# brentp/goleft

Measured on AMD Instinct MI355X. Metric: ref bases/sec per-base depth, 30x WGS synthetic, higher is better.
Workload: dtype int32; 1 GPU; synthetic 30x WGS, hg19 contig lengths (3.1 Gb), 150 bp reads; window=1000, min_mapq=1, min_cov=4, total_ref_bases=3095677412, reads_rank0=619135482, cigar_ops_rank0=687232250, canonical_cigar_ops_rank0=0, tiles_on_the_generic_kernel=24, step=gd_compute on the records as they arrived (nothing derived exists), outputs=int32 per-base depth + int64/int32 window sum/min + class runs, tile_positions=4096, lookback=192

## Files before the change

### goleft_amd/csrc/gd_kernels.hpp

```cpp
#pragma once

#include <hip/hip_runtime.h>
#include <stdint.h>

namespace gd {

constexpr int WAVE = 64;
constexpr int SUPER = 1024;

struct ContigDev {
    const int32_t*  pos;
    const uint16_t* flag;
    const uint8_t*  mapq;
    const uint32_t* off;
    const uint32_t* cigar;
    uint32_t n_reads;
    uint32_t n_ops;
    int32_t  length;
    int32_t  tile_beg;
    int32_t  n_tiles;
    int64_t  base_off;
    int64_t  win_off;
    int32_t  tid;
    uint32_t unit_beg;
    uint32_t grp_beg;
    const uint4*    lrec;
    const uint32_t* lfq;
    const uint2*    dl;
    const uint32_t* pck;
    const uint32_t* ndel;
    const uint32_t* rec;
    const uint32_t* pidx;
    uint32_t pidx_last;
    uint32_t pad_;
};

struct __attribute__((aligned(16))) TileInfo {
    const int32_t*  pos;
    const uint16_t* flag;
    const uint8_t*  mapq;
    const uint32_t* off;
    const uint32_t* cigar;
    int64_t  base_off;
    int64_t  win_off;
    int32_t  length;
    int32_t  ctg;
    int32_t  t0;
    uint32_t lo, hi;
    uint32_t n_reads;
    uint32_t n_ops;
    uint32_t clo, chi;
    int32_t  tile;
    int32_t  pad_;
    const uint32_t* ndel;
    const uint4*    lrec;
    const uint32_t* lfq;
    const uint2*    dl;
    const uint32_t* pck;
};

struct __attribute__((aligned(16))) TileFast {
    const int32_t*  pos;
    const uint32_t* rec;
    const uint32_t* cig;
    const uint16_t* flag;
    const uint8_t*  mapq;
    int32_t*  out;
    int64_t*  wsum;
    int32_t*  wmin;
    int32_t   t0;
    uint32_t  nrd;
    uint32_t  nst;
    uint32_t  clo;
    int32_t   ctg;
    int32_t   pad_[3];
    uint32_t  win0[4];
    int32_t   wleft[4];
    int32_t   sleft[4];
};
constexpr int FAST_BIG = 0x3fffffff;
constexpr int FAST_FAR = FAST_BIG - 65536;

struct Counters {
    int32_t  max_span;
    uint32_t run_cursor;
    uint32_t pad0;
    uint32_t pad1;
    uint32_t n_slow[2];
    uint32_t pad2[2];
};

struct Job {
    const ContigDev* ctgs;
    int32_t   n_ctgs;
    int32_t   n_tiles;
    TileInfo* tiles;
    int32_t*  perbase;
    int64_t*  win_sum;
    int32_t*  win_min;
    int64_t   n_win_total;
    int2*     run_chunks;
    uint32_t  run_cap;
    uint32_t* tile_cnt;
    uint32_t* tile_off;
    uint32_t* super_cnt;
    Counters* counters;
    int32_t   W;
    int32_t   Q;
    int32_t   mincov;
    int32_t   maxmean;
    uint32_t  flag_mask;
    int32_t   lookback;
    int32_t   reserved0;
    int64_t   step;
    uint32_t  n_units;
    uint32_t  n_groups;
    unsigned long long* tile_status;
    uint32_t  w_magic, w_shift;
    uint32_t  s_magic, s_shift;
    uint32_t  fast;
    uint32_t  parity;
    TileFast* ftiles;
};

__device__ __forceinline__ int cov_class(int d, int mincov, int maxmean)
{
    int c = 2;
    if (maxmean > 0 && d >= maxmean) c = 3;
    if (d < mincov) c = 1;
    if (d == 0) c = 0;
    return c;
}

__device__ __forceinline__ uint32_t lower_bound_i32(const int32_t* a, uint32_t n, int32_t key)
{
    uint32_t lo = 0, hi = n;
    while (lo < hi) {
        uint32_t mid = lo + ((hi - lo) >> 1);
        if (a[mid] < key) lo = mid + 1; else hi = mid;
    }
    return lo;
}

__device__ __forceinline__ void lower_bound_pair(const int32_t* a, uint32_t n, int32_t keyA,
                                                 int32_t keyB, uint32_t& outA, uint32_t& outB)
{
    uint32_t la = 0, ha = n, lb = 0, hb = n;
    if (n == 0) { outA = 0; outB = 0; return; }
    const uint32_t last = n - 1;
    while (ha > la || hb > lb) {
        const uint32_t wa = ha - la, wb = hb - lb;
        uint32_t a1 = la + (wa >> 2), a2 = la + (wa >> 1), a3 = la + wa - (wa >> 2) - (wa != 0);
        uint32_t b1 = lb + (wb >> 2), b2 = lb + (wb >> 1), b3 = lb + wb - (wb >> 2) - (wb != 0);
        a1 = a1 < last ? a1 : last; a2 = a2 < last ? a2 : last; a3 = a3 < last ? a3 : last;
        b1 = b1 < last ? b1 : last; b2 = b2 < last ? b2 : last; b3 = b3 < last ? b3 : last;
        const int32_t va1 = a[a1], va2 = a[a2], va3 = a[a3];
        const int32_t vb1 = a[b1], vb2 = a[b2], vb3 = a[b3];
        if (wa != 0) {
            if (va3 < keyA) la = a3 + 1;
            else if (va2 < keyA) { la = a2 + 1; ha = a3; }
            else if (va1 < keyA) { la = a1 + 1; ha = a2; }
            else ha = a1;
        }
        if (wb != 0) {
            if (vb3 < keyB) lb = b3 + 1;
            else if (vb2 < keyB) { lb = b2 + 1; hb = b3; }
            else if (vb1 < keyB) { lb = b1 + 1; hb = b2; }
            else hb = b1;
        }
    }
    outA = la;
    outB = lb;
}

__device__ __forceinline__ uint32_t lower_bound_hint(const int32_t* a, uint32_t n, int32_t key, uint32_t guess)
{
    if (n == 0u) return 0u;
    constexpr uint32_t R = 8192u;
    const uint32_t g = guess < n ? guess : n - 1u;
    const uint32_t pl = g > R ? g - R : 0u;
    const uint32_t ph = n - 1u - g > R ? g + R : n - 1u;
    const int32_t vl = a[pl], vh = a[ph];
    uint32_t lo = 0, hi = n;
    if (vl < key) {
        lo = pl + 1u;
        if (vh >= key) hi = ph; else lo = ph + 1u;
    } else {
        hi = pl;
    }
    while (lo < hi) {
        const uint32_t mid = lo + ((hi - lo) >> 1);
        if (a[mid] < key) lo = mid + 1u; else hi = mid;
    }
    return lo;
}

template <int T>
__global__ void gd_prep_kernel(Job job)
{
    const int64_t gid = (int64_t)blockIdx.x * blockDim.x + threadIdx.x;
    const int64_t gsz = (int64_t)gridDim.x * blockDim.x;
    for (int64_t w = gid; w < job.n_win_total; w += gsz) {
        job.win_sum[w] = 0;
        job.win_min[w] = 0x7fffffff;
    }
    for (int64_t g = gid; g < (job.n_tiles + SUPER - 1) / SUPER; g += gsz) job.super_cnt[g] = 0;
    const int32_t lookback = job.lookback;
    if (gid == 0) {
        job.counters->max_span = 0;
        job.counters->run_cursor = 0;
        job.counters->n_slow[job.parity ^ 1u] = 0;
    }
    if (gid >= job.n_tiles) return;
    const int t = (int)gid;
    int lo = 0, hi = job.n_ctgs;
    while (hi - lo > 1) {
        int mid = (lo + hi) >> 1;
        if (job.ctgs[mid].tile_beg <= t) lo = mid; else hi = mid;
    }
    const ContigDev c = job.ctgs[lo];
    TileInfo ti;
    ti.pos = c.pos; ti.flag = c.flag; ti.mapq = c.mapq; ti.off = c.off; ti.cigar = c.cigar;
    ti.base_off = c.base_off; ti.win_off = c.win_off; ti.length = c.length;
    ti.n_reads = c.n_reads; ti.n_ops = c.n_ops;
    ti.ctg = lo;
    ti.tile = t;
    ti.pad_ = 0;
    ti.ndel = c.ndel;
    ti.lrec = c.lrec; ti.lfq = c.lfq; ti.dl = c.dl; ti.pck = c.pck;
    ti.t0 = (t - c.tile_beg) * T;
    int32_t tend = ti.t0 + T < c.length ? ti.t0 + T : c.length;
    int32_t from = ti.t0 > lookback ? ti.t0 - lookback : 0;
    if (c.pidx) {
        const uint32_t kl = (uint32_t)from >> 6, k = (uint32_t)tend >> 6;
        ti.lo = kl > c.pidx_last ? c.n_reads : c.pidx[kl];
        const uint32_t a = k > c.pidx_last ? c.n_reads : c.pidx[k];
        ti.hi = (tend & 63) == 0 ? a : a + lower_bound_i32(c.pos + a, (k + 1u > c.pidx_last ? c.n_reads : c.pidx[k + 1]) - a, tend);
    } else {
        const uint32_t n = c.n_reads;
        const uint32_t g0 = (uint32_t)(((uint64_t)(uint32_t)ti.t0 * n) / (uint32_t)c.length);
        const uint32_t s0 = ti.t0 == 0 ? 0u : lower_bound_hint(c.pos, n, ti.t0, g0);
        const uint32_t nxt = (uint32_t)__shfl_down((int)s0, 1, WAVE);
        const int tnx = __shfl_down(t, 1, WAVE);
        const bool have = (threadIdx.x & 63u) != 63u && t + 1 < job.n_tiles && tnx == t + 1 &&
                          t + 1 - c.tile_beg < c.n_tiles && ti.t0 + T == tend;
        if (have) ti.hi = nxt;
        else {
            const uint32_t g1 = (uint32_t)(((uint64_t)(uint32_t)tend * n) / (uint32_t)c.length);
            ti.hi = lower_bound_hint(c.pos + s0, n - s0, tend, g1 > s0 ? g1 - s0 : 0u) + s0;
        }
        uint32_t lo = 0, hi2 = s0;
        if (from == 0) hi2 = 0u;
        for (uint32_t step = 64u; hi2 > 0u; step <<= 2) {
            const uint32_t p = hi2 > step ? hi2 - step : 0u;
            if (c.pos[p] >= from) hi2 = p; else { lo = p + 1u; break; }
        }
        while (lo < hi2) {
            const uint32_t mid = lo + ((hi2 - lo) >> 1);
            if (c.pos[mid] < from) lo = mid + 1u; else hi2 = mid;
        }
        ti.lo = lo;
    }
    if (job.fast == 2u) ti.lo &= ~3u;
    ti.clo = c.n_reads ? c.off[ti.lo] : 0u;
    ti.chi = c.n_reads ? c.off[ti.hi] : 0u;
    if (!job.fast) { job.tiles[t] = ti; return; }
    TileFast tf;
    const uint32_t nrd = ti.hi - ti.lo, nst = ti.chi - ti.clo;
    const bool ordinary = tend - ti.t0 == T && nrd <= 1024u && nst <= (job.fast == 2u ? 1280u : 1024u);
    tf.nrd = 0xffffffffu;
    if (ordinary) {
        tf.pos = c.pos + ti.lo; tf.cig = c.cigar + ti.clo;
        if (job.fast == 2u) { tf.rec = c.off + ti.lo; tf.flag = c.flag + ti.lo; tf.mapq = c.mapq + ti.lo; }
        else { tf.rec = c.rec + ti.lo; tf.flag = nullptr; tf.mapq = nullptr; }
        tf.out = job.perbase ? job.perbase + c.base_off + ti.t0 : nullptr;
        tf.wsum = job.win_sum + c.win_off;
        tf.wmin = job.win_min + c.win_off;
        tf.t0 = ti.t0; tf.nrd = nrd; tf.nst = nst; tf.clo = ti.clo; tf.ctg = lo;
        tf.pad_[0] = tf.pad_[1] = tf.pad_[2] = 0;
        const uint32_t W = (uint32_t)job.W;
        const uint32_t stepc = job.step > 0x7fffffffLL ? 0x7fffffffu : (uint32_t)job.step;
#pragma unroll
        for (int w = 0; w < 4; ++w) {
            const uint32_t cpos0 = (uint32_t)ti.t0 + (uint32_t)(w * (T / 4));
            const uint32_t cw = cpos0 / W, wleft = W - (cpos0 - cw * W);
            const uint32_t srem = cpos0 % stepc, sleft = srem == 0u ? 0u : stepc - srem;
            tf.win0[w] = cw;
            tf.wleft[w] = wleft > (uint32_t)FAST_FAR ? FAST_BIG : (int32_t)wleft;
            tf.sleft[w] = sleft > (uint32_t)FAST_FAR ? FAST_BIG : (int32_t)sleft;
        }
    } else {
        const uint32_t slot = atomicAdd(&job.counters->n_slow[job.parity], 1u);
        job.tiles[slot] = ti;
    }
    job.ftiles[t] = tf;
}

__global__ __launch_bounds__(64) void gd_copy_words_kernel(const uint32_t* __restrict__ src, uint32_t* __restrict__ dst, uint32_t n)
{
    for (uint32_t i = threadIdx.x; i < n; i += 64u) dst[i] = src[i];
}

__global__ __launch_bounds__(256) void gd_readback_kernel(const Counters* __restrict__ k, const int2* __restrict__ ordered, uint32_t spec,
                                                          Counters* __restrict__ h_counters, int2* __restrict__ h_bounds)
{
    const uint32_t n = k->run_cursor < spec ? k->run_cursor : spec;
    for (uint32_t i = threadIdx.x; i < n; i += 256u) h_bounds[i] = ordered[i];
    if (threadIdx.x < sizeof(Counters) / 4u)
        reinterpret_cast<uint32_t*>(h_counters)[threadIdx.x] = reinterpret_cast<const uint32_t*>(k)[threadIdx.x];
}

__device__ __forceinline__ int wave_inclusive_scan(int v)
{
    v += __builtin_amdgcn_update_dpp(0, v, 0x111, 0xf, 0xf, false);
    v += __builtin_amdgcn_update_dpp(0, v, 0x112, 0xf, 0xf, false);
    v += __builtin_amdgcn_update_dpp(0, v, 0x114, 0xf, 0xf, false);
    v += __builtin_amdgcn_update_dpp(0, v, 0x118, 0xf, 0xf, false);
    v += __builtin_amdgcn_update_dpp(0, v, 0x142, 0xa, 0xf, false);
    v += __builtin_amdgcn_update_dpp(0, v, 0x143, 0xc, 0xf, false);
    return v;
}

__device__ __forceinline__ void scan4(int& a, int& b, int& c, int& d)
{
#define GD_DPP4(ctl)                                  \
    "v_add_u32_dpp %0, %0, %0 " ctl "\n\t"            \
    "v_add_u32_dpp %1, %1, %1 " ctl "\n\t"            \
    "v_add_u32_dpp %2, %2, %2 " ctl "\n\t"            \
    "v_add_u32_dpp %3, %3, %3 " ctl "\n\t"
    asm volatile(
        "s_nop 1\n\t"
        GD_DPP4("row_shr:1 row_mask:0xf bank_mask:0xf bound_ctrl:1")
        GD_DPP4("row_shr:2 row_mask:0xf bank_mask:0xf bound_ctrl:1")
        GD_DPP4("row_shr:4 row_mask:0xf bank_mask:0xf bound_ctrl:1")
        GD_DPP4("row_shr:8 row_mask:0xf bank_mask:0xf bound_ctrl:1")
        GD_DPP4("row_bcast:15 row_mask:0xa bank_mask:0xf")
        GD_DPP4("row_bcast:31 row_mask:0xc bank_mask:0xf")
        : "+v"(a), "+v"(b), "+v"(c), "+v"(d));
#undef GD_DPP4
}

__device__ __forceinline__ int wave_sum(int v)
{
#pragma unroll
    for (int m = 32; m >= 1; m >>= 1) v += __shfl_xor(v, m, WAVE);
    return v;
}

__device__ __forceinline__ long long wave_sum64(long long v)
{
#pragma unroll
    for (int m = 32; m >= 1; m >>= 1) v += __shfl_xor(v, m, WAVE);
    return v;
}

__device__ __forceinline__ int wave_min(int v)
{
#pragma unroll
    for (int m = 32; m >= 1; m >>= 1) {
        int o = __shfl_xor(v, m, WAVE);
        v = o < v ? o : v;
    }
    return v;
}

struct RegionTab {
    const int32_t* depth;
    int64_t  clen, start, end;
    int64_t  first_win;
    uint32_t win_off;
    uint32_t chunk_off;
};
constexpr int REGION_CHUNK = 4096;

__global__ __launch_bounds__(256) void gd_regions_windows_kernel(const RegionTab* __restrict__ tab,
                                                                 const uint32_t* __restrict__ win_region, int32_t W,
                                                                 int64_t* __restrict__ sums, int32_t* __restrict__ mins)
{
    __shared__ long long s_sum[4];
    __shared__ int s_min[4];
    const uint32_t w = blockIdx.x;
    const RegionTab t = tab[win_region[w]];
    const int64_t k = t.first_win + (int64_t)(w - t.win_off);
    int64_t ws = k * W, we = ws + W;
    if (ws < t.start) ws = t.start;
    if (we > t.end) we = t.end;
    long long acc = 0;
    int mn = 0x7fffffff;
    for (int64_t p = ws + threadIdx.x; p < we; p += 256) {
        const int d = p < t.clen ? t.depth[p] : 0;
        acc += d;
        mn = d < mn ? d : mn;
    }
    acc = wave_sum64(acc);
    mn = wave_min(mn);
    const int lane = threadIdx.x & 63, wv = threadIdx.x >> 6;
    if (lane == 0) { s_sum[wv] = acc; s_min[wv] = mn; }
    __syncthreads();
    if (threadIdx.x == 0) {
        int m = s_min[0];
        for (int i = 1; i < 4; ++i) m = s_min[i] < m ? s_min[i] : m;
        sums[w] = s_sum[0] + s_sum[1] + s_sum[2] + s_sum[3];
        mins[w] = m;
    }
}

__global__ __launch_bounds__(256) void gd_regions_bounds_kernel(const RegionTab* __restrict__ tab,
                                                                const uint32_t* __restrict__ chunk_region, int mincov,
                                                                int maxmean, int4* __restrict__ out, uint32_t cap,
                                                                uint32_t* __restrict__ cursor)
{
    const uint32_t ch = blockIdx.x;
    const uint32_t r = chunk_region[ch];
    const RegionTab t = tab[r];
    const int64_t p0 = t.start + (int64_t)(ch - t.chunk_off) * REGION_CHUNK;
    const int64_t p1 = p0 + REGION_CHUNK < t.end ? p0 + REGION_CHUNK : t.end;
    for (int64_t p = p0 + threadIdx.x; p < p1; p += 256) {
        const int d = p < t.clen ? t.depth[p] : 0;
        const int cl = cov_class(d, mincov, maxmean);
        bool b = (p == t.start);
        if (!b) {
            const int dp = (p - 1) < t.clen ? t.depth[p - 1] : 0;
// ... 144 lines not shown
```

### goleft_amd/csrc/gd_tile_common.hpp

```cpp
#pragma once

#include <type_traits>

namespace gd {

typedef __amdgpu_buffer_rsrc_t rsrc_t;

__device__ __forceinline__ rsrc_t make_rsrc(const void* p, uint32_t bytes)
{
    return __builtin_amdgcn_make_buffer_rsrc(const_cast<void*>(p), (short)0, (int)bytes, 0x00020000);
}

__device__ __forceinline__ int wave_total(int v)
{
    return __builtin_amdgcn_readlane(wave_inclusive_scan(v), 63);
}

__device__ __forceinline__ int wave_prev_lane(int v, int first)
{
    return __builtin_amdgcn_update_dpp(first, v, 0x138, 0xf, 0xf, false);
}

__device__ __forceinline__ int wave_min_dpp(int v)
{
    int o;
    o = __builtin_amdgcn_update_dpp(v, v, 0x111, 0xf, 0xf, false); v = o < v ? o : v;
    o = __builtin_amdgcn_update_dpp(v, v, 0x112, 0xf, 0xf, false); v = o < v ? o : v;
    o = __builtin_amdgcn_update_dpp(v, v, 0x114, 0xf, 0xf, false); v = o < v ? o : v;
    o = __builtin_amdgcn_update_dpp(v, v, 0x118, 0xf, 0xf, false); v = o < v ? o : v;
    o = __builtin_amdgcn_update_dpp(v, v, 0x142, 0xa, 0xf, false); v = o < v ? o : v;
    o = __builtin_amdgcn_update_dpp(v, v, 0x143, 0xc, 0xf, false); v = o < v ? o : v;
    return __builtin_amdgcn_readlane(v, 63);
}

__device__ __forceinline__ uint32_t wave_max_dpp(uint32_t v)
{
    uint32_t o;
    o = (uint32_t)__builtin_amdgcn_update_dpp((int)v, (int)v, 0x111, 0xf, 0xf, false); v = o > v ? o : v;
    o = (uint32_t)__builtin_amdgcn_update_dpp((int)v, (int)v, 0x112, 0xf, 0xf, false); v = o > v ? o : v;
    o = (uint32_t)__builtin_amdgcn_update_dpp((int)v, (int)v, 0x114, 0xf, 0xf, false); v = o > v ? o : v;
    o = (uint32_t)__builtin_amdgcn_update_dpp((int)v, (int)v, 0x118, 0xf, 0xf, false); v = o > v ? o : v;
    o = (uint32_t)__builtin_amdgcn_update_dpp((int)v, (int)v, 0x142, 0xa, 0xf, false); v = o > v ? o : v;
    o = (uint32_t)__builtin_amdgcn_update_dpp((int)v, (int)v, 0x143, 0xc, 0xf, false); v = o > v ? o : v;
    return (uint32_t)__builtin_amdgcn_readlane((int)v, 63);
}

__device__ __forceinline__ void publish_span(int32_t* max_span, uint32_t smax, int seen0, int lane)
{
    if (__builtin_amdgcn_ballot_w64(smax > (uint32_t)seen0) != 0ull) {
        const uint32_t m = wave_max_dpp(smax);
        if (lane == 0) atomicMax(max_span, (int32_t)m);
    }
}

__device__ __forceinline__ int32_t* lds_at(int32_t* base, int b4)
{
    return reinterpret_cast<int32_t*>(reinterpret_cast<char*>(base) + b4);
}

__device__ __forceinline__ void mark4(int32_t* s_diff, int s4, int e4, int T4)
{
    if (e4 >= 0) {
        const int cs4 = s4 > -4 ? s4 : -4;
        atomicAdd(lds_at(s_diff, cs4), 1);
        if (e4 < T4) atomicAdd(lds_at(s_diff, e4), -1);
    }
}

constexpr uint32_t SPAN_SAT = 1u << 28;

template <typename OpPtr>
__device__ __forceinline__ uint32_t walk_cigar4(OpPtr ops, uint32_t n, int ps4, int T4, int32_t* s_diff)
{
    uint32_t span = 0;
    for (uint32_t k = 0; k < n; ++k) {
        const uint32_t cg = ops[k];
        const uint32_t op = cg & 0xf, len = cg >> 4;
        const bool counted = (0x181u >> op) & 1u;
        const bool consumes = (0x18du >> op) & 1u;
        if (counted && len != 0 && span < SPAN_SAT) {
            const int s4 = ps4 + (int)(span << 2);
            if (s4 < T4) mark4(s_diff, s4, s4 + (int)(len << 2), T4);
        }
        if (consumes) { span += len; span = span < SPAN_SAT ? span : SPAN_SAT; }
    }
    return span;
}

struct PhaseA {
    const int32_t* pos; const uint16_t* flag; const uint8_t* mapq; const uint32_t* off;
    int32_t* s_diff;
    const uint32_t* s_cig;
    uint32_t* wq;
    const uint32_t* gcig;
    uint32_t clo, nrd;
    int neg4t0, T4;
    uint32_t flag_mask;
    int Q, tid, lane;
};

struct PhaseB {
    int32_t* s_diff;
    uint32_t* s_bmap; uint32_t* s_clo; uint32_t* s_chi; uint32_t* s_hasb;
    int32_t* out;
    int64_t* wsum; int32_t* wmin;
    int t0, tlen, chunk0, carry, lane;
    int W, mincov, maxmean;
    int64_t step;
};

template <int ROWS, bool FULL, bool WIDE, int ST>
__device__ __forceinline__ void phase_b_rows(const PhaseB& B)
{
    constexpr int BIG = 0x3fffffff;
    typedef typename std::conditional<WIDE, unsigned long long, uint32_t>::type acc_t;
    const int lane = B.lane, t0 = B.t0, tlen = B.tlen, chunk0 = B.chunk0;
    const int W = B.W;
    int carry = B.carry;

    const uint32_t cpos0 = (uint32_t)t0 + (uint32_t)chunk0;
    uint32_t cur_win = cpos0 / (uint32_t)W;
    const int64_t nb_abs = ((int64_t)cur_win + 1) * (int64_t)W;
    int nb = (nb_abs - t0) > BIG ? BIG : (int)(nb_abs - t0);
    const uint32_t stepc = B.step > 0x7fffffffLL ? 0x7fffffffu : (uint32_t)B.step;
    const int64_t nf_abs = (int64_t)((cpos0 + stepc - 1) / stepc) * (int64_t)stepc;
    int nf = (nf_abs - t0) > BIG ? BIG : (int)(nf_abs - t0);
    const int wstep = W > BIG ? BIG : W;
    const int fstep = stepc > (uint32_t)BIG ? BIG : (int)stepc;
    acc_t acc = 0;
    int mn = 0x7fffffff;
    const int lo_thr = B.mincov > 1 ? B.mincov : 1;
    const int hi_thr = B.maxmean > 0 ? B.maxmean : 0x7fffffff;
    const bool has_max = B.maxmean > 0;

#pragma unroll
    for (int r = 0; r < ROWS; ++r) {
        const int rb = chunk0 + r * 256;
        const int ib = rb + lane * 4;
        int4* dst = reinterpret_cast<int4*>(&B.out[ib]);
        if (!FULL && rb >= tlen) {
            if (ST != 2) *dst = make_int4(0, 0, 0, 0);
            continue;
        }
        const int4 v = *reinterpret_cast<const int4*>(&B.s_diff[ib]);
        const int x1 = v.x + v.y, x2 = x1 + v.z, x3 = x2 + v.w;
        const int incl = wave_inclusive_scan(x3);
        const int base = carry + (incl - x3);
        int d0 = base + v.x, d1 = base + x1, d2 = base + x2, d3 = base + x3;
        const int carry_before = carry;
        carry += __builtin_amdgcn_readlane(incl, 63);
        int nvalid = 4;
        if (!FULL) {
            nvalid = tlen - ib;
            nvalid = nvalid < 0 ? 0 : (nvalid > 4 ? 4 : nvalid);
            d0 = nvalid > 0 ? d0 : 0; d1 = nvalid > 1 ? d1 : 0;
            d2 = nvalid > 2 ? d2 : 0; d3 = nvalid > 3 ? d3 : 0;
        }
        if (ST == 2) {
        } else if (ST == 1) {
            typedef int v4i32 __attribute__((ext_vector_type(4)));
            v4i32 dv; dv.x = d0; dv.y = d1; dv.z = d2; dv.w = d3;
            __builtin_nontemporal_store(dv, reinterpret_cast<v4i32*>(dst));
        } else {
            *dst = make_int4(d0, d1, d2, d3);
        }

        const uint32_t s4 = (uint32_t)d0 + (uint32_t)d1 + (uint32_t)d2 + (uint32_t)d3;
        int t = d0 < d1 ? d0 : d1;
        t = d2 < t ? d2 : t;
        t = d3 < t ? d3 : t;

        if (FULL && nb >= rb + 256) {
            acc += s4;
            mn = t < mn ? t : mn;
        } else if (FULL && !WIDE && nb + wstep >= rb + 256) {
            const int rel = nb - rb;
            const int L = rel >> 2, k = rel & 3;
            const bool lt = lane < L;
            const uint32_t a_old = (uint32_t)acc + (lt ? s4 : 0u);
            const int t_old = lt ? t : 0x7fffffff;
            const int m_old = t_old < mn ? t_old : mn;
            const int e0 = __builtin_amdgcn_readlane(d0, L), e1 = __builtin_amdgcn_readlane(d1, L);
            const int e2 = __builtin_amdgcn_readlane(d2, L), e3 = __builtin_amdgcn_readlane(d3, L);
            const uint32_t ps = (k > 0 ? (uint32_t)e0 : 0u) + (k > 1 ? (uint32_t)e1 : 0u) +
                                (k > 2 ? (uint32_t)e2 : 0u);
            int pm = 0x7fffffff;
            if (k > 0) pm = e0 < pm ? e0 : pm;
            if (k > 1) pm = e1 < pm ? e1 : pm;
            if (k > 2) pm = e2 < pm ? e2 : pm;
            const uint32_t qs = (uint32_t)e0 + (uint32_t)e1 + (uint32_t)e2 + (uint32_t)e3 - ps;
            int qm = e3;
            if (k <= 0) qm = e0 < qm ? e0 : qm;
            if (k <= 1) qm = e1 < qm ? e1 : qm;
            if (k <= 2) qm = e2 < qm ? e2 : qm;
            const uint32_t tot = (uint32_t)wave_total((int)a_old) + ps;
            int m = wave_min_dpp(m_old);
            m = pm < m ? pm : m;
            if (lane == 0) {
                atomicAdd(reinterpret_cast<unsigned long long*>(&B.wsum[cur_win]),
                          (unsigned long long)tot);
                atomicMin(&B.wmin[cur_win], m);
            }
            const bool gt = lane > L;
            acc = gt ? s4 : 0u;
            mn = gt ? t : 0x7fffffff;
            if (lane == L) { acc = qs; mn = qm; }
            cur_win++;
            nb = nb + wstep > BIG ? BIG : nb + wstep;
        } else {
            int seg = rb;
            const int dd[4] = {d0, d1, d2, d3};
            while (nb < rb + 256 && nb < tlen) {
#pragma unroll
                for (int j = 0; j < 4; ++j) {
                    const int pj = ib + j;
                    if (pj >= seg && pj < nb) { acc += (uint32_t)dd[j]; mn = dd[j] < mn ? dd[j] : mn; }
                }
                const long long tot = wave_sum64((long long)acc);
                const int m = wave_min(mn);
                if (lane == 0) {
                    atomicAdd(reinterpret_cast<unsigned long long*>(&B.wsum[cur_win]),
                              (unsigned long long)tot);
                    atomicMin(&B.wmin[cur_win], m);
                }
                acc = 0; mn = 0x7fffffff;
                cur_win++; seg = nb;
                nb = nb + wstep > BIG ? BIG : nb + wstep;
            }
#pragma unroll
            for (int j = 0; j < 4; ++j) {
                const int pj = ib + j;
                if (pj >= seg && j < nvalid) { acc += (uint32_t)dd[j]; mn = dd[j] < mn ? dd[j] : mn; }
            }
        }

// ... 103 lines not shown
```

### goleft_amd/csrc/gd_tile_fast.hpp

```cpp
#pragma once

#ifndef GD_LOAD_AUX
#define GD_LOAD_AUX 0
#endif

namespace gd {
namespace fast {

constexpr int T = 4096;
constexpr int NT = 256;
constexpr int NW = NT / WAVE;
constexpr int CHUNK = T / NW;
constexpr int ROWS = CHUNK / 256;
constexpr int CQ = 1280;
constexpr int U = 4;
constexpr int QCAP = 120;
constexpr int NWORDS = T / 32;

template <int ST>
__global__ __launch_bounds__(NT) void gd_tile_fast_kernel(Job job)
{
    constexpr int CQN = CQ;
    constexpr int QCAPN = QCAP;
    __shared__ __attribute__((aligned(16))) int32_t s_diffp[T + 4];
    __shared__ __attribute__((aligned(16))) uint32_t s_cig[CQN];
    __shared__ uint32_t s_q[3 * QCAPN];
    __shared__ int32_t  s_wtot[NW];
    __shared__ uint32_t s_wcnt[NW];
    __shared__ uint32_t s_qn;
    __shared__ uint32_t s_hasb;
    __shared__ uint32_t s_base;
    int32_t* const s_diff = s_diffp + 4;
    uint32_t* const s_bmap = s_cig;
    uint32_t* const s_clo = s_cig + NWORDS;
    uint32_t* const s_chi = s_cig + 2 * NWORDS;

    const int per = (job.n_tiles + 7) >> 3;
    const int tile = (int)(blockIdx.x & 7u) * per + (int)(blockIdx.x >> 3);
    if (tile >= job.n_tiles) return;
    const TileFast* __restrict__ const tp = job.ftiles + tile;
    struct {
        const int32_t* pos; const uint32_t* rec; const uint32_t* cig; const uint16_t* flag; const uint8_t* mapq;
        int32_t* out; int64_t* wsum; int32_t* wmin; int32_t t0; uint32_t nrd, nst, clo; int32_t ctg;
    } tf;
    tf.nrd = tp->nrd;
    if ((int32_t)tf.nrd < 0) return;
    tf.pos = tp->pos; tf.rec = tp->rec; tf.cig = tp->cig;
    tf.flag = tp->flag; tf.mapq = tp->mapq; tf.clo = tp->clo;
    tf.out = tp->out; tf.wsum = tp->wsum; tf.wmin = tp->wmin;
    tf.t0 = tp->t0; tf.nst = tp->nst; tf.ctg = tp->ctg;

    const int tid = threadIdx.x;
    const int lane = tid & (WAVE - 1);
    const int wv = __builtin_amdgcn_readfirstlane(tid >> 6);
    const int seen0 = __hip_atomic_load(&job.counters->max_span, __ATOMIC_RELAXED, __HIP_MEMORY_SCOPE_AGENT);
    constexpr int T4 = T * 4;

    const uint32_t nrd = tf.nrd;
    const rsrc_t r_pos = make_rsrc(tf.pos, nrd * 4u);
    const rsrc_t r_rec = make_rsrc(tf.rec, (nrd != 0u ? nrd + 1u : nrd) * 4u);
    const rsrc_t r_cig = make_rsrc(tf.cig, tf.nst * 4u);
    const int tid4 = tid * 4;
    typedef unsigned int v4u __attribute__((ext_vector_type(4)));
    typedef unsigned int v2u __attribute__((ext_vector_type(2)));
    const v4u pv = __builtin_amdgcn_raw_buffer_load_b128(r_pos, tid * 16, 0, GD_LOAD_AUX);
    const v4u rv = __builtin_amdgcn_raw_buffer_load_b128(r_rec, tid * 16, 0, GD_LOAD_AUX);
    const rsrc_t r_flag = make_rsrc(tf.flag, ((nrd + 1u) & ~1u) * 2u);
    const rsrc_t r_mapq = make_rsrc(tf.mapq, (nrd + 3u) & ~3u);
    const uint32_t o4 = (uint32_t)__builtin_amdgcn_raw_buffer_load_b32(r_rec, tid * 16 + 16, 0, GD_LOAD_AUX);
    const v2u fv = __builtin_amdgcn_raw_buffer_load_b64(r_flag, tid * 8, 0, GD_LOAD_AUX);
    const uint32_t mv = (uint32_t)__builtin_amdgcn_raw_buffer_load_b32(r_mapq, tid4, 0, GD_LOAD_AUX);
    uint32_t cgv[CQN / NT];
#pragma unroll
    for (int k = 0; k < CQN / NT; ++k)
        cgv[k] = (uint32_t)__builtin_amdgcn_raw_buffer_load_b32(r_cig, tid4 + k * NT * 4, 0, GD_LOAD_AUX);

    {
        const int4 z = make_int4(0, 0, 0, 0);
        int4* d4 = reinterpret_cast<int4*>(s_diffp);
#pragma unroll
        for (int i = 0; i < T / 4 / NT; ++i) d4[tid + i * NT] = z;
        if (tid == 0) { d4[T / 4] = z; s_qn = 0; s_hasb = 0; }
    }
    const uint32_t rec[U] = {rv.x, rv.y, rv.z, rv.w};
    uint32_t n[U], ex[U];
    {
        const uint32_t oe[U] = {rv.y, rv.z, rv.w, o4};
#pragma unroll
        for (int u = 0; u < U; ++u) {
            n[u] = (uint32_t)(tid4 + u) < nrd ? oe[u] - rec[u] : 0u;
            ex[u] = rec[u] - tf.clo;
        }
    }
#pragma unroll
    for (int k = 0; k < CQN / NT; ++k) s_cig[k * NT + tid] = cgv[k];
    __syncthreads();

    uint32_t smax = 0;
    {
        const int neg4t0 = (int)(0u - ((uint32_t)tf.t0 << 2));
        const int32_t p[U] = {(int32_t)pv.x, (int32_t)pv.y, (int32_t)pv.z, (int32_t)pv.w};
        uint32_t cg[U], idx[U];
        bool keep[U];
#pragma unroll
        for (int u = 0; u < U; ++u) {
            idx[u] = ex[u];
            const uint32_t fw = u < 2 ? fv.x : fv.y;
            const uint32_t f = (u & 1) ? fw >> 16 : fw & 0xffffu;
            const uint32_t mq = (mv >> (8 * u)) & 0xffu;
            keep[u] = ((f & job.flag_mask) == 0) & ((int)mq >= job.Q) & (n[u] != 0);
        }
#pragma unroll
        for (int u = 0; u < U; ++u) cg[u] = s_cig[keep[u] ? idx[u] : 0u];
        uint32_t cg2[U];
#pragma unroll
        for (int u = 0; u < U; ++u) {
            const uint32_t x = s_cig[(keep[u] & (n[u] == 2u)) ? idx[u] + 1u : 0u];
            cg2[u] = n[u] == 2u ? x : 0u;
        }
        int ps4[U];
        bool cx[U];
#pragma unroll
        for (int u = 0; u < U; ++u) {
            ps4[u] = (int)(((uint32_t)p[u] << 2) + (uint32_t)neg4t0);
            {
                const uint32_t oa = cg[u] & 0xfu, la = cg[u] >> 4, ob = cg2[u] & 0xfu, lb = cg2[u] >> 4;
                const bool ca = (0x181u >> oa) & 1u, ka = (0x18du >> oa) & 1u;
                const bool cb = (0x181u >> ob) & 1u, kb = (0x18du >> ob) & 1u;
                const bool simple = keep[u] & (n[u] <= 2u);
                cx[u] = keep[u] & (n[u] > 2u);
                uint32_t L = (ca ? la : 0u) + (cb ? lb : 0u);
                const uint32_t so = (ka & !ca) ? la : 0u;
                const uint32_t span = (ka ? la : 0u) + (kb ? lb : 0u);
                const uint32_t rs = simple ? (span < SPAN_SAT ? span : SPAN_SAT) : 0u;
                smax = rs > smax ? rs : smax;
                L = L < (1u << 27) ? L : (1u << 27);
                const int s4 = ps4[u] + (int)(so << 2);
                const int e4 = s4 + (int)(L << 2);
                if (simple & (L != 0u) & (e4 >= 0) & (s4 < T4)) {
                    const int cs4 = s4 > -4 ? s4 : -4;
                    atomicAdd(lds_at(s_diff, cs4), 1);
                    if (e4 < T4) atomicAdd(lds_at(s_diff, e4), -1);
                }
            }
        }
        unsigned long long m[U];
        uint32_t cnt[U];
#pragma unroll
        for (int u = 0; u < U; ++u) { m[u] = __builtin_amdgcn_ballot_w64(cx[u]); cnt[u] = (uint32_t)__popcll(m[u]); }
        const uint32_t tot = cnt[0] + cnt[1] + cnt[2] + cnt[3];
        if (tot != 0u) {
            uint32_t b = 0;
            if (lane == 0) b = atomicAdd(&s_qn, tot);
            b = (uint32_t)__builtin_amdgcn_readfirstlane((int)b);
#pragma unroll
            for (int u = 0; u < U; ++u) {
                if (cx[u]) {
                    const uint32_t rk = b + __builtin_amdgcn_mbcnt_hi((uint32_t)(m[u] >> 32),
                                                __builtin_amdgcn_mbcnt_lo((uint32_t)m[u], 0u));
                    if (rk < (uint32_t)QCAPN) {
                        s_q[rk] = (uint32_t)ps4[u]; s_q[QCAPN + rk] = idx[u]; s_q[2 * QCAPN + rk] = n[u];
                    } else {
                        const uint32_t sp = walk_cigar4(s_cig + idx[u], n[u], ps4[u], T4, s_diff);
                        smax = sp > smax ? sp : smax;
                    }
                }
                b += cnt[u];
            }
        }
    }
    __syncthreads();

    {
        const uint32_t nq = s_qn < (uint32_t)QCAPN ? s_qn : (uint32_t)QCAPN;
        if ((uint32_t)(wv * WAVE) < nq) {
            if ((uint32_t)tid < nq) {
                const uint32_t sp = walk_cigar4(s_cig + s_q[QCAPN + tid], s_q[2 * QCAPN + tid], (int)s_q[tid], T4, s_diff);
                smax = sp > smax ? sp : smax;
            }
        }
        publish_span(&job.counters->max_span, smax, seen0, lane);
    }
    __syncthreads();

    const int chunk0 = wv * CHUNK;
    int4 v[ROWS];
#pragma unroll
    for (int r = 0; r < ROWS; ++r)
        v[r] = *reinterpret_cast<const int4*>(&s_diff[chunk0 + r * 256 + lane * 4]);
    s_cig[tid] = 0;
    if (tid < 3 * NWORDS - NT) s_cig[NT + tid] = 0;
    int x1[ROWS], x2[ROWS], x3[ROWS], incl[ROWS];
#pragma unroll
    for (int r = 0; r < ROWS; ++r) {
        x1[r] = v[r].x + v[r].y; x2[r] = x1[r] + v[r].z; x3[r] = x2[r] + v[r].w;
        incl[r] = x3[r];
    }
    scan4(incl[0], incl[1], incl[2], incl[3]);
    int rtot[ROWS];
#pragma unroll
    for (int r = 0; r < ROWS; ++r) rtot[r] = __builtin_amdgcn_readlane(incl[r], 63);
    if (lane == 0) s_wtot[wv] = rtot[0] + rtot[1] + rtot[2] + rtot[3];
    __syncthreads();

    {
        constexpr int BIG = FAST_BIG;
        int carry = s_diff[-1];
#pragma unroll
        for (int w = 0; w < NW - 1; ++w) carry += w < wv ? s_wtot[w] : 0;
        int cin[ROWS + 1];
        cin[0] = carry;
#pragma unroll
        for (int r = 0; r < ROWS; ++r) cin[r + 1] = cin[r] + rtot[r];
        int d[ROWS][4];
        uint32_t s4[ROWS];
        int t[ROWS];
        int32_t* const out = tf.out;
#pragma unroll
        for (int r = 0; r < ROWS; ++r) {
            const int base = cin[r] + (incl[r] - x3[r]);
            d[r][0] = base + v[r].x; d[r][1] = base + x1[r]; d[r][2] = base + x2[r]; d[r][3] = base + x3[r];
            if (ST != 2) {
                int4* dst = reinterpret_cast<int4*>(&out[chunk0 + r * 256 + lane * 4]);
                if (ST == 1) {
                    typedef int v4i32 __attribute__((ext_vector_type(4)));
                    v4i32 dv; dv.x = d[r][0]; dv.y = d[r][1]; dv.z = d[r][2]; dv.w = d[r][3];
                    __builtin_nontemporal_store(dv, reinterpret_cast<v4i32*>(dst));
                } else {
                    *dst = make_int4(d[r][0], d[r][1], d[r][2], d[r][3]);
                }
            }
            s4[r] = (uint32_t)d[r][0] + (uint32_t)d[r][1] + (uint32_t)d[r][2] + (uint32_t)d[r][3];
            int m = d[r][0] < d[r][1] ? d[r][0] : d[r][1];
            m = d[r][2] < m ? d[r][2] : m;
            t[r] = d[r][3] < m ? d[r][3] : m;
        }

        const int W = job.W;
        uint32_t cur_win = tp->win0[wv];
        const int wl = tp->wleft[wv], sl = tp->sleft[wv];
        int nb = wl >= BIG ? BIG : chunk0 + wl;
        int nf = sl >= BIG ? BIG : chunk0 + sl;
        const int wstep = W > FAST_FAR ? BIG : W;
        const uint32_t stepc = job.step > 0x7fffffffLL ? 0x7fffffffu : (uint32_t)job.step;
        const int fstep = stepc > (uint32_t)FAST_FAR ? BIG : (int)stepc;
        uint32_t acc = 0;
        int mn = 0x7fffffff;
        const int lo_thr = job.mincov > 1 ? job.mincov : 1;
        const int hi_thr = job.maxmean > 0 ? job.maxmean : 0x7fffffff;
        const bool has_max = job.maxmean > 0;
        int64_t* const wsum = tf.wsum;
        int32_t* const wmin = tf.wmin;

        bool any_noisy;
        {
            int tm = t[0];
#pragma unroll
            for (int r = 1; r < ROWS; ++r) tm = t[r] < tm ? t[r] : tm;
            any_noisy = __builtin_amdgcn_ballot_w64(tm < lo_thr) != 0ull;
            if (has_max) {
                int tx = d[0][0];
#pragma unroll
                for (int r = 0; r < ROWS; ++r) {
#pragma unroll
                    for (int j = 0; j < 4; ++j) tx = d[r][j] > tx ? d[r][j] : tx;
                }
                any_noisy = any_noisy || __builtin_amdgcn_ballot_w64(tx >= hi_thr) != 0ull;
            }
            any_noisy = any_noisy || carry < lo_thr || carry >= hi_thr || nf < chunk0 + ROWS * 256;
        }

#pragma unroll
        for (int r = 0; r < ROWS; ++r) {
            const int rb = chunk0 + r * 256;
            const int ib = rb + lane * 4;
            const int d0 = d[r][0], d1 = d[r][1], d2 = d[r][2], d3 = d[r][3];

            if (nb >= rb + 256) {
                acc += s4[r];
                mn = t[r] < mn ? t[r] : mn;
            } else if (nb + wstep >= rb + 256) {
                const int rel = nb - rb;
                const int L = rel >> 2, k = rel & 3;
                const bool lt = lane < L;
                const uint32_t a_old = acc + (lt ? s4[r] : 0u);
                const int t_old = lt ? t[r] : 0x7fffffff;
                const int m_old = t_old < mn ? t_old : mn;
                const int e0 = __builtin_amdgcn_readlane(d0, L), e1 = __builtin_amdgcn_readlane(d1, L);
                const int e2 = __builtin_amdgcn_readlane(d2, L), e3 = __builtin_amdgcn_readlane(d3, L);
                const uint32_t ps = (k > 0 ? (uint32_t)e0 : 0u) + (k > 1 ? (uint32_t)e1 : 0u) +
                                    (k > 2 ? (uint32_t)e2 : 0u);
                int pm = 0x7fffffff;
                if (k > 0) pm = e0 < pm ? e0 : pm;
                if (k > 1) pm = e1 < pm ? e1 : pm;
                if (k > 2) pm = e2 < pm ? e2 : pm;
                const uint32_t qs = (uint32_t)e0 + (uint32_t)e1 + (uint32_t)e2 + (uint32_t)e3 - ps;
                int qm = e3;
                if (k <= 0) qm = e0 < qm ? e0 : qm;
                if (k <= 1) qm = e1 < qm ? e1 : qm;
                if (k <= 2) qm = e2 < qm ? e2 : qm;
                const uint32_t tot = (uint32_t)wave_total((int)a_old) + ps;
                int m = wave_min_dpp(m_old);
                m = pm < m ? pm : m;
                if (lane == 0) {
                    atomicAdd(reinterpret_cast<unsigned long long*>(&wsum[cur_win]), (unsigned long long)tot);
                    atomicMin(&wmin[cur_win], m);
                }
                const bool gt = lane > L;
                acc = gt ? s4[r] : 0u;
                mn = gt ? t[r] : 0x7fffffff;
                if (lane == L) { acc = qs; mn = qm; }
                cur_win++;
                nb = nb + wstep > BIG ? BIG : nb + wstep;
            } else {
                int seg = rb;
                const int dd[4] = {d0, d1, d2, d3};
                while (nb < rb + 256) {
#pragma unroll
                    for (int j = 0; j < 4; ++j) {
                        const int pj = ib + j;
                        if (pj >= seg && pj < nb) { acc += (uint32_t)dd[j]; mn = dd[j] < mn ? dd[j] : mn; }
                    }
                    const uint32_t tot = (uint32_t)wave_total((int)acc);
                    const int m = wave_min_dpp(mn);
                    if (lane == 0) {
                        atomicAdd(reinterpret_cast<unsigned long long*>(&wsum[cur_win]), (unsigned long long)tot);
                        atomicMin(&wmin[cur_win], m);
                    }
                    acc = 0; mn = 0x7fffffff;
                    cur_win++; seg = nb;
                    nb = nb + wstep > BIG ? BIG : nb + wstep;
                }
#pragma unroll
                for (int j = 0; j < 4; ++j) {
                    const int pj = ib + j;
                    if (pj >= seg) { acc += (uint32_t)dd[j]; mn = dd[j] < mn ? dd[j] : mn; }
                }
            }

            if (any_noisy) {
                const int carry_before = cin[r];
                bool noisy = __ballot(t[r] < lo_thr) != 0ull;
                if (has_max) {
                    int tx = d0 > d1 ? d0 : d1;
                    tx = d2 > tx ? d2 : tx;
                    tx = d3 > tx ? d3 : tx;
                    noisy = noisy || __ballot(tx >= hi_thr) != 0ull;
                }
                noisy = noisy || carry_before < lo_thr || carry_before >= hi_thr;
                if (noisy || nf < rb + 256) {
                    const int pl = wave_prev_lane(d3, carry_before);
                    const int c0 = cov_class(d0, job.mincov, job.maxmean);
                    const int c1 = cov_class(d1, job.mincov, job.maxmean);
                    const int c2 = cov_class(d2, job.mincov, job.maxmean);
                    const int c3 = cov_class(d3, job.mincov, job.maxmean);
                    const int cp = cov_class(pl, job.mincov, job.maxmean);
                    uint32_t bm = (uint32_t)(c0 != cp) | ((uint32_t)(c1 != c0) << 1) |
                                  ((uint32_t)(c2 != c1) << 2) | ((uint32_t)(c3 != c2) << 3);
                    while (nf < rb + 256) {
                        const int o = nf - ib;
                        if (o >= 0 && o < 4) bm |= 1u << o;
                        nf = nf + fstep > BIG ? BIG : nf + fstep;
                    }
                    if (__ballot(bm != 0) != 0ull) {
                        if (bm != 0) {
                            const uint32_t lo = ((uint32_t)(c0 & 1)) | ((uint32_t)(c1 & 1) << 1) |
                                                ((uint32_t)(c2 & 1) << 2) | ((uint32_t)(c3 & 1) << 3);
                            const uint32_t hi = ((uint32_t)(c0 >> 1)) | ((uint32_t)(c1 >> 1) << 1) |
                                                ((uint32_t)(c2 >> 1) << 2) | ((uint32_t)(c3 >> 1) << 3);
                            const int w = ib >> 5, sh = ib & 31;
                            atomicOr(&s_bmap[w], bm << sh);
                            atomicOr(&s_clo[w], (lo & bm) << sh);
                            atomicOr(&s_chi[w], (hi & bm) << sh);
                        }
// ... 22 lines not shown
```

Before: 817.4 billion ref-bases/s.

## Pack the per-base difference array into biased 16-bit halves in LDS

The fast tile kernel's LDS difference array now stores two positions per 32-bit word as biased 16-bit counters, updated with shifted atomic adds, instead of one int32 per position. Decoding during the prefix scan reconstructs per-position deltas with carry-corrected arithmetic. This halves the LDS footprint and the clear/read traffic, so more workgroups fit per CU. It relies on static bounds on marks per tile to avoid 16-bit overflow, and adds decode arithmetic in the scan.

```diff
diff --git a/goleft_amd/csrc/gd_kernels.hpp b/goleft_amd/csrc/gd_kernels.hpp
--- a/goleft_amd/csrc/gd_kernels.hpp
+++ b/goleft_amd/csrc/gd_kernels.hpp
@@ -78,6 +78,9 @@
     int32_t   wleft[4];
     int32_t   sleft[4];
 };
+constexpr uint32_t FAST_MAX_READS = 1024;
+constexpr uint32_t FAST_MAX_OPS_RAW = 1280;
+constexpr uint32_t FAST_MAX_OPS = 1024;
 constexpr int FAST_BIG = 0x3fffffff;
 constexpr int FAST_FAR = FAST_BIG - 65536;
 
@@ -267,7 +270,7 @@
     if (!job.fast) { job.tiles[t] = ti; return; }
     TileFast tf;
     const uint32_t nrd = ti.hi - ti.lo, nst = ti.chi - ti.clo;
-    const bool ordinary = tend - ti.t0 == T && nrd <= 1024u && nst <= (job.fast == 2u ? 1280u : 1024u);
+    const bool ordinary = tend - ti.t0 == T && nrd <= FAST_MAX_READS && nst <= (job.fast == 2u ? FAST_MAX_OPS_RAW : FAST_MAX_OPS);
     tf.nrd = 0xffffffffu;
     if (ordinary) {
         tf.pos = c.pos + ti.lo; tf.cig = c.cigar + ti.clo;
diff --git a/goleft_amd/csrc/gd_tile_common.hpp b/goleft_amd/csrc/gd_tile_common.hpp
--- a/goleft_amd/csrc/gd_tile_common.hpp
+++ b/goleft_amd/csrc/gd_tile_common.hpp
@@ -81,6 +81,45 @@
         if (counted && len != 0 && span < SPAN_SAT) {
             const int s4 = ps4 + (int)(span << 2);
             if (s4 < T4) mark4(s_diff, s4, s4 + (int)(len << 2), T4);
+        }
+        if (consumes) { span += len; span = span < SPAN_SAT ? span : SPAN_SAT; }
+    }
+    return span;
+}
+
+constexpr int PK_BIAS = 0x4000;
+constexpr int PK_MAX_MARKS = PK_BIAS;
+
+template <int V>
+__device__ __forceinline__ void mark_packed1(uint32_t* s_diff, int p2)
+{
+    static_assert(V == 1 || V == -1, "a mark");
+    uint32_t* const w = reinterpret_cast<uint32_t*>(reinterpret_cast<char*>(s_diff) + (p2 & ~3));
+    uint32_t val;
+    asm("v_lshlrev_b32_e64 %0, %1, %2" : "=v"(val) : "v"((uint32_t)p2 << 3), "n"(V));
+    atomicAdd(w, val);
+}
+
+__device__ __forceinline__ void mark_packed(uint32_t* s_diff, int s2, int e2, int T2)
+{
+    if (e2 >= 0) {
+        mark_packed1<1>(s_diff, s2 > -2 ? s2 : -2);
+        if (e2 < T2) mark_packed1<-1>(s_diff, e2);
+    }
+}
+
+template <typename OpPtr>
+__device__ __forceinline__ uint32_t walk_cigar_packed(OpPtr ops, uint32_t n, int ps2, int T2, uint32_t* s_diff)
+{
+    uint32_t span = 0;
+    for (uint32_t k = 0; k < n; ++k) {
+        const uint32_t cg = ops[k];
+        const uint32_t op = cg & 0xf, len = cg >> 4;
+        const bool counted = (0x181u >> op) & 1u;
+        const bool consumes = (0x18du >> op) & 1u;
+        if (counted && len != 0 && span < SPAN_SAT) {
+            const int s2 = ps2 + (int)(span << 1);
+            if (s2 < T2) mark_packed(s_diff, s2, s2 + (int)(len << 1), T2);
         }
         if (consumes) { span += len; span = span < SPAN_SAT ? span : SPAN_SAT; }
     }
diff --git a/goleft_amd/csrc/gd_tile_fast.hpp b/goleft_amd/csrc/gd_tile_fast.hpp
--- a/goleft_amd/csrc/gd_tile_fast.hpp
+++ b/goleft_amd/csrc/gd_tile_fast.hpp
@@ -16,13 +16,21 @@
 constexpr int U = 4;
 constexpr int QCAP = 120;
 constexpr int NWORDS = T / 32;
+constexpr int LDS_BYTES = (T / 2 + 4) * 4 + CQ * 4 + 3 * QCAP * 4 + 2 * NW * 4 + 3 * 4;
+static_assert(LDS_BYTES * 8 <= 160 * 1024, "eight workgroups per CU");
+
+static_assert((uint32_t)CQ == FAST_MAX_OPS_RAW, "the staging area holds exactly the ops of an ordinary tile");
+static_assert(FAST_MAX_READS <= (uint32_t)CQ, "every candidate read of an ordinary tile has a staged op");
+static_assert(FAST_MAX_READS <= (uint32_t)PK_MAX_MARKS, "candidate reads of an ordinary tile vs the packed 16-bit entries");
+static_assert(CQ <= PK_MAX_MARKS, "staged ops (queue walk and the over-QCAP in-place walk mark from them) vs the packed 16-bit entries");
+static_assert(QCAP <= CQ && FAST_MAX_READS == (uint32_t)(NT * U), "one batch: every lane takes U reads");
 
 template <int ST>
 __global__ __launch_bounds__(NT) void gd_tile_fast_kernel(Job job)
 {
     constexpr int CQN = CQ;
     constexpr int QCAPN = QCAP;
-    __shared__ __attribute__((aligned(16))) int32_t s_diffp[T + 4];
+    __shared__ __attribute__((aligned(16))) uint32_t s_diffp[T / 2 + 4];
     __shared__ __attribute__((aligned(16))) uint32_t s_cig[CQN];
     __shared__ uint32_t s_q[3 * QCAPN];
     __shared__ int32_t  s_wtot[NW];
@@ -30,7 +38,7 @@
     __shared__ uint32_t s_qn;
     __shared__ uint32_t s_hasb;
     __shared__ uint32_t s_base;
-    int32_t* const s_diff = s_diffp + 4;
+    uint32_t* const s_diff = s_diffp + 4;
     uint32_t* const s_bmap = s_cig;
     uint32_t* const s_clo = s_cig + NWORDS;
     uint32_t* const s_chi = s_cig + 2 * NWORDS;
@@ -54,7 +62,7 @@
     const int lane = tid & (WAVE - 1);
     const int wv = __builtin_amdgcn_readfirstlane(tid >> 6);
     const int seen0 = __hip_atomic_load(&job.counters->max_span, __ATOMIC_RELAXED, __HIP_MEMORY_SCOPE_AGENT);
-    constexpr int T4 = T * 4;
+    constexpr int T2 = T * 2;
 
     const uint32_t nrd = tf.nrd;
     const rsrc_t r_pos = make_rsrc(tf.pos, nrd * 4u);
@@ -76,11 +84,12 @@
         cgv[k] = (uint32_t)__builtin_amdgcn_raw_buffer_load_b32(r_cig, tid4 + k * NT * 4, 0, GD_LOAD_AUX);
 
     {
-        const int4 z = make_int4(0, 0, 0, 0);
+        const int4 z = make_int4(PK_BIAS, PK_BIAS, PK_BIAS, PK_BIAS);
         int4* d4 = reinterpret_cast<int4*>(s_diffp);
-#pragma unroll
-        for (int i = 0; i < T / 4 / NT; ++i) d4[tid + i * NT] = z;
-        if (tid == 0) { d4[T / 4] = z; s_qn = 0; s_hasb = 0; }
+        static_assert((T / 2) % (4 * NT) == 0, "whole vectors per thread");
+#pragma unroll
+        for (int i = 0; i < T / 8 / NT; ++i) d4[tid + i * NT] = z;
+        if (tid == 0) { d4[T / 8] = z; s_qn = 0; s_hasb = 0; }
     }
     const uint32_t rec[U] = {rv.x, rv.y, rv.z, rv.w};
     uint32_t n[U], ex[U];
@@ -98,7 +107,7 @@
 
     uint32_t smax = 0;
     {
-        const int neg4t0 = (int)(0u - ((uint32_t)tf.t0 << 2));
+        const int neg2t0 = (int)(0u - ((uint32_t)tf.t0 << 1));
         const int32_t p[U] = {(int32_t)pv.x, (int32_t)pv.y, (int32_t)pv.z, (int32_t)pv.w};
         uint32_t cg[U], idx[U];
         bool keep[U];
@@ -118,11 +127,11 @@
             const uint32_t x = s_cig[(keep[u] & (n[u] == 2u)) ? idx[u] + 1u : 0u];
             cg2[u] = n[u] == 2u ? x : 0u;
         }
-        int ps4[U];
+        int ps2[U];
         bool cx[U];
 #pragma unroll
         for (int u = 0; u < U; ++u) {
-            ps4[u] = (int)(((uint32_t)p[u] << 2) + (uint32_t)neg4t0);
+            ps2[u] = (int)(((uint32_t)p[u] << 1) + (uint32_t)neg2t0);
             {
                 const uint32_t oa = cg[u] & 0xfu, la = cg[u] >> 4, ob = cg2[u] & 0xfu, lb = cg2[u] >> 4;
                 const bool ca = (0x181u >> oa) & 1u, ka = (0x18du >> oa) & 1u;
@@ -135,12 +144,11 @@
                 const uint32_t rs = simple ? (span < SPAN_SAT ? span : SPAN_SAT) : 0u;
                 smax = rs > smax ? rs : smax;
                 L = L < (1u << 27) ? L : (1u << 27);
-                const int s4 = ps4[u] + (int)(so << 2);
-                const int e4 = s4 + (int)(L << 2);
-                if (simple & (L != 0u) & (e4 >= 0) & (s4 < T4)) {
-                    const int cs4 = s4 > -4 ? s4 : -4;
-                    atomicAdd(lds_at(s_diff, cs4), 1);
-                    if (e4 < T4) atomicAdd(lds_at(s_diff, e4), -1);
+                const int s2 = ps2[u] + (int)(so << 1);
+                const int e2 = s2 + (int)(L << 1);
+                if (simple & (L != 0u) & (e2 >= 0) & (s2 < T2)) {
+                    mark_packed1<1>(s_diff, s2 > -2 ? s2 : -2);
+                    if (e2 < T2) mark_packed1<-1>(s_diff, e2);
                 }
             }
         }
@@ -159,9 +167,9 @@
                     const uint32_t rk = b + __builtin_amdgcn_mbcnt_hi((uint32_t)(m[u] >> 32),
                                                 __builtin_amdgcn_mbcnt_lo((uint32_t)m[u], 0u));
                     if (rk < (uint32_t)QCAPN) {
-                        s_q[rk] = (uint32_t)ps4[u]; s_q[QCAPN + rk] = idx[u]; s_q[2 * QCAPN + rk] = n[u];
+                        s_q[rk] = (uint32_t)ps2[u]; s_q[QCAPN + rk] = idx[u]; s_q[2 * QCAPN + rk] = n[u];
                     } else {
-                        const uint32_t sp = walk_cigar4(s_cig + idx[u], n[u], ps4[u], T4, s_diff);
+                        const uint32_t sp = walk_cigar_packed(s_cig + idx[u], n[u], ps2[u], T2, s_diff);
                         smax = sp > smax ? sp : smax;
                     }
                 }
@@ -175,7 +183,7 @@
         const uint32_t nq = s_qn < (uint32_t)QCAPN ? s_qn : (uint32_t)QCAPN;
         if ((uint32_t)(wv * WAVE) < nq) {
             if ((uint32_t)tid < nq) {
-                const uint32_t sp = walk_cigar4(s_cig + s_q[QCAPN + tid], s_q[2 * QCAPN + tid], (int)s_q[tid], T4, s_diff);
+                const uint32_t sp = walk_cigar_packed(s_cig + s_q[QCAPN + tid], s_q[2 * QCAPN + tid], (int)s_q[tid], T2, s_diff);
                 smax = sp > smax ? sp : smax;
             }
         }
@@ -184,16 +192,18 @@
     __syncthreads();
 
     const int chunk0 = wv * CHUNK;
-    int4 v[ROWS];
+    int2 v[ROWS];
 #pragma unroll
     for (int r = 0; r < ROWS; ++r)
-        v[r] = *reinterpret_cast<const int4*>(&s_diff[chunk0 + r * 256 + lane * 4]);
+        v[r] = *reinterpret_cast<const int2*>(&s_diff[(chunk0 + r * 256 + lane * 4) >> 1]);
     s_cig[tid] = 0;
     if (tid < 3 * NWORDS - NT) s_cig[NT + tid] = 0;
-    int x1[ROWS], x2[ROWS], x3[ROWS], incl[ROWS];
+    int h0[ROWS], h1[ROWS], y1[ROWS], x3[ROWS], incl[ROWS];
 #pragma unroll
     for (int r = 0; r < ROWS; ++r) {
-        x1[r] = v[r].x + v[r].y; x2[r] = x1[r] + v[r].z; x3[r] = x2[r] + v[r].w;
+        h0[r] = v[r].x >> 16; h1[r] = v[r].y >> 16;
+        y1[r] = v[r].x - 65535 * h0[r];
+        x3[r] = (v[r].y - 65535 * h1[r]) + y1[r] - 2 * PK_BIAS;
         incl[r] = x3[r];
     }
     scan4(incl[0], incl[1], incl[2], incl[3]);
@@ -205,7 +215,7 @@
 
     {
         constexpr int BIG = FAST_BIG;
-        int carry = s_diff[-1];
+        int carry = (int)s_diff[-1] >> 16;
 #pragma unroll
         for (int w = 0; w < NW - 1; ++w) carry += w < wv ? s_wtot[w] : 0;
         int cin[ROWS + 1];
@@ -219,7 +229,8 @@
 #pragma unroll
         for (int r = 0; r < ROWS; ++r) {
             const int base = cin[r] + (incl[r] - x3[r]);
-            d[r][0] = base + v[r].x; d[r][1] = base + x1[r]; d[r][2] = base + x2[r]; d[r][3] = base + x3[r];
+            d[r][3] = base + x3[r]; d[r][2] = d[r][3] - h1[r];
+            d[r][1] = base + y1[r] - PK_BIAS; d[r][0] = d[r][1] - h0[r];
             if (ST != 2) {
                 int4* dst = reinterpret_cast<int4*>(&out[chunk0 + r * 256 + lane * 4]);
                 if (ST == 1) {
```

Measured after the change: 812.4 billion ref-bases/s. Within noise of the previous version (-0.6%).
